# jdfxzzy/DPMN

Measured on AMD Instinct MI355X. Metric: SR images/sec (16x64->32x128, bs=48 per GPU, fp32 forward), higher is better.
Workload: dtype f32; 1 GPU; cfg1: TATT PSN + 3+3 PGRM (embed 96, windows 2/4/8) + CMM, forward-only; per_gpu_batch=48, global_batch=48, ranks=1, batches_in_flight=2, parallelism=dp1 (independent batch shards, no forward collective)

## Files before the change

### dpmn_amd/_abi.py

```python
import ctypes as C
import os

import torch

_HERE = os.path.dirname(os.path.abspath(__file__))
LIB_PATH = os.environ.get("DPMN_HIP_LIB") or os.path.join(_HERE, "lib", "libdpmn_hip.so")

if not os.path.exists(LIB_PATH):
    raise RuntimeError(
        "dpmn_amd: %s not found -- build it with `python -c 'import __graft_entry__ as g; g.build()'` "
        "(or `make -C dpmn_amd/csrc`).  There is no CPU fallback for the DPMN hot path." % LIB_PATH)

lib = C.CDLL(LIB_PATH)

fp = C.c_void_p


class PgrmBlock(C.Structure):
    _fields_ = [(n, fp) for n in (
        "norm1_q_w", "norm1_q_b", "norm1_kv_w", "norm1_kv_b", "q_w", "q_b", "kv_w", "kv_b")] + [
        ("bias_table", fp * 4)] + [(n, fp) for n in (
            "sk_proj_w", "sk_proj_b", "sk_fc1_w", "sk_fc1_b", "sk_fc2_w", "sk_fc2_b", "sk_head_w", "sk_head_b",
            "norm2_w", "norm2_b", "fc1_w", "fc1_b", "dw_w", "dw_b", "pw_w", "pw_b", "fc2_w", "fc2_b")]

# ... 118 lines not shown
    "dpmn_distill_forward_f32": (_i, [C.POINTER(DistillParams), fp, fp, _i, fp, fp, fp, fp, fp, _sz, _i, _i, _i, fp]),
    "dpmn_distill_backward_f32": (_i, [C.POINTER(DistillParams), C.POINTER(DistillGrads), fp, fp, fp, fp, fp, fp, fp, fp, fp, _sz, _i, _i, _i, fp]),
    "dpmn_conv2d_wgrad_unpack_multi_f32": (_i, [fp, fp, _i, _i, fp]),
    "dpmn_tl_interp_f32": (_i, [fp, fp, _i, _i, _i, _i, _i, fp]),
    "dpmn_pointwise_wgrad_det_bytes": (_sz, [_i, _i]),
    "dpmn_reduce_defer_begin": (_i, []),
    "dpmn_reduce_defer_enable": (_i, [_i]),
    "dpmn_reduce_defer_push": (_i, [C.POINTER(TnPending)]),
    "dpmn_reduce_defer_pending": (_i, []),
    "dpmn_reduce_defer_flush": (_i, [_i, fp]),
    "dpmn_xred_fallbacks": (_i, [C.POINTER(C.c_uint), _i]),
    "dpmn_selftest_xshfl": (_i, [C.POINTER(C.c_uint)]),
    "dpmn_selftest_lds_poison": (_i, [C.c_uint, _i, fp]),
    "dpmn_xred_test_force_recompute": (_i, [_i]),
    "dpmn_xred_enable": (_i, [_i]),
    "dpmn_nchw_to_nhwc_f32": (_i, [fp, fp, _i, _i, _i, _i, _i, fp]),
    "dpmn_nhwc_to_nchw_f32": (_i, [fp, fp, _i, _i, _i, _i, fp]),
    "dpmn_se_gate_f32": (_i, [fp, fp, fp, fp, fp, fp, fp, _i, _i, _i, _i, fp]),
    "dpmn_bigru_f32": (_i, [fp, fp, fp, fp, fp, _i, _i, _i, C.c_long, C.c_long, C.c_long, _i, fp]),
    "dpmn_small_linear_f32": (_i, [fp, fp, _i, fp, fp, fp, _i, _i, _i, _i, _f, fp]),
    "dpmn_tatt_encoder_layer_f32": (_i, [fp, fp, _PP, fp, _i, _i, _i, _i, fp]),
    "dpmn_cross_attn_f32": (_i, [fp, fp, fp, fp, fp, _i, _i, _i, _i, _i, fp]),
    "dpmn_add_layernorm64_f32": (_i, [fp, fp, fp, fp, fp, fp, fp, fp, _f, _i, C.c_long, fp]),
    "dpmn_gru_gate_f32": (_i, [fp, fp, fp, fp, C.c_long, _i, _i, fp]),
    "dpmn_to_mask_f32": (_i, [fp, C.c_long, fp, _i, _i, _i, fp]),
    "dpmn_mha32_f32": (_i, [fp, fp, _i, _i, _i, _f, fp]),
    "dpmn_layernorm_std_f32": (_i, [fp, fp, fp, _f, fp, _l, _i, fp]),
    "dpmn_rotate_img_f32": (_i, [fp, fp, fp, _f, fp, _i, _i, _i, _i, fp]),
    "dpmn_blend_f32": (_i, [fp, C.c_long, fp, C.c_long, fp, _f, _i, _i, fp]),
    "dpmn_psnr_ssim_workspace_bytes": (_sz, [_i, _i, _i, _i]),
    "dpmn_psnr_ssim_f32": (_i, [fp, C.c_long, fp, C.c_long, fp, fp, _i, _i, _i, _i, fp]),
    "dpmn_gemm_tn_f32": (_i, [fp, fp, fp, fp, _i, _i, _i, fp, _sz, fp]),
    "dpmn_gemm_tn_partial_bytes": (_sz, [_i, _i, _i]),
    "dpmn_gemm_tn_partial_f32": (_i, [fp, fp, fp, fp, _i, _i, _i, fp, _sz, C.POINTER(TnPending), fp]),
    "dpmn_tn_reduce_multi_f32": (_i, [C.POINTER(TnPending), _i, fp]),
    "dpmn_gemm_tn_group_f32": (_i, [C.POINTER(TnItem), _i, fp]),
    "dpmn_colsum_f32": (_i, [fp, fp, C.c_long, _i, fp]),
    "dpmn_colsum_det_f32": (_i, [fp, fp, C.c_long, _i, fp, _sz, fp]),
    "dpmn_layernorm_bwd_f32": (_i, [fp, fp, fp, _f, fp, _i, fp, fp, C.c_long, _i, fp]),
    "dpmn_layernorm_bwd_det_f32": (_i, [fp, fp, fp, _f, fp, _i, fp, fp, C.c_long, _i, fp, _sz, fp]),
    "dpmn_layernorm_bwd_det_drop_f32": (_i, [fp, fp, fp, _f, fp, _i, fp, fp, C.c_long, _i, fp, _sz, fp, _f, _u64, _f, _u64, _l, fp]),
    "dpmn_layernorm_f32": (_i, [fp, fp, fp, _f, fp, C.c_long, _i, fp]),
    "dpmn_act_bwd_f32": (_i, [fp, fp, fp, _i, _f, C.c_long, fp]),
    "dpmn_act_fwd_f32": (_i, [fp, fp, _i, _f, C.c_long, fp]),
    "dpmn_axpby_f32": (_i, [fp, fp, fp, _f, _f, _i, C.c_long, fp]),
    "dpmn_rowsum_mod_f32": (_i, [fp, fp, C.c_long, _i, _i, fp]),
# ... 234 lines not shown
```

### dpmn_amd/csrc/common.h

```cpp
#pragma once
#include <hip/hip_runtime.h>
#include <stdint.h>
#include <atomic>
#include "../../include/dpmn_hip.h"

typedef float f32x4 __attribute__((ext_vector_type(4)));

#define DPMN_CHECK_LAUNCH()                                                         \
  do {                                                                              \
    hipError_t e__ = hipGetLastError();                                             \
    if (e__ != hipSuccess) return dpmn_set_error(DPMN_ERR_LAUNCH, hipGetErrorString(e__)); \
  } while (0)

#define DPMN_REQUIRE(cond, msg)                                    \
  do {                                                             \
    if (!(cond)) return dpmn_set_error(DPMN_ERR_ARG, msg);         \
  } while (0)

int dpmn_set_error(int code, const char* msg);

__device__ __forceinline__ f32x4 mfma16(float a, float b, f32x4 c) {
  return __builtin_amdgcn_mfma_f32_16x16x4f32(a, b, c, 0, 0, 0);
}

// ... 121 lines not shown
  return u >= p ? inv_keep : 0.0f;
}
__device__ __forceinline__ float drop_scale(unsigned long long seed, unsigned long long idx, float p, float inv_keep) {
  return drop_scale_z(drop_z0(seed, idx), p, inv_keep);
}

static inline hipStream_t as_stream(dpmn_stream_t s) { return (hipStream_t)s; }

constexpr int DPMN_MAX_DEVICES = 64;
int dpmn_cu_count();
template <auto Kernel>
inline void dpmn_lds_optin(size_t bytes) {
  static std::atomic<int> set[DPMN_MAX_DEVICES];
  int dev = -1;
  const bool keyed = hipGetDevice(&dev) == hipSuccess && dev >= 0 && dev < DPMN_MAX_DEVICES;
  if (keyed && (int)bytes <= set[dev].load(std::memory_order_relaxed)) return;
  if (hipFuncSetAttribute(reinterpret_cast<const void*>(Kernel), hipFuncAttributeMaxDynamicSharedMemorySize, (int)bytes) == hipSuccess && keyed)
    set[dev].store((int)bytes, std::memory_order_relaxed);
}

enum ProfTag { PT_CONV_IGEMM_128 = 0, PT_CONV_IGEMM_64, PT_CONV_IGEMM_NARROW, PT_CONV_SPLITK_REDUCE, PT_CONV_HALO, PT_CONV_HALO_C4,
               PT_GEMM_PW, PT_GEMM_WSTAT, PT_GEMM_KLOOP, PT_DWCONV_GELU, PT_WATTN8, PT_WATTN_SCALAR, PT_ATTN_FUSED, PT_BIGRU,
               PT_MHA32, PT_PATCH_EMBED, PT_SK_GATE, PT_TAIL, PT_GEMM_WSTAT_LN, PT_CONV_IGEMM_SK, PT_ATTN_FUSED_BWD, PT_WATTN_BWD,
               PT_CONV_WGRAD, PT_GEMM_TN, PT_TN_REDUCE, PT_DWCONV_BWD, PT_WGRAD_UNPACK, PT_CONV_PACK, PT_AFFINE_ACT_BWD, PT_LN_BWD, PT_WATTN_MFMA32, PT_COUNT };
extern unsigned long long g_dpmn_prof_mask;
extern double g_dpmn_prof_hint_bytes;
extern int g_dpmn_bf16;
extern int g_dpmn_x3;
typedef __bf16 bf16x2 __attribute__((ext_vector_type(2)));
typedef __bf16 bf16x8 __attribute__((ext_vector_type(8)));
__device__ __forceinline__ uint2 pack_bf16x4(float a, float b, float c, float d) {
  typedef float f32x2_ __attribute__((ext_vector_type(2)));
  const bf16x2 lo = __builtin_convertvector((f32x2_){a, b}, bf16x2), hi = __builtin_convertvector((f32x2_){c, d}, bf16x2);
  return make_uint2(__builtin_bit_cast(unsigned, lo), __builtin_bit_cast(unsigned, hi));
}
__device__ __forceinline__ f32x4 mfma16_bf16(bf16x8 a, bf16x8 b, f32x4 c) {
  return __builtin_amdgcn_mfma_f32_16x16x32_bf16(a, b, c, 0, 0, 0);
}
__device__ __forceinline__ void x3_split2t(float a, float b, unsigned& h, unsigned& m, unsigned& l) {
  const unsigned ua = __float_as_uint(a), ub = __float_as_uint(b);
  h = __builtin_amdgcn_perm(ub, ua, 0x07060302u);
  const float ra = a - __uint_as_float(ua & 0xffff0000u), rb = b - __uint_as_float(ub & 0xffff0000u);
  const unsigned va = __float_as_uint(ra), vb = __float_as_uint(rb);
  m = __builtin_amdgcn_perm(vb, va, 0x07060302u);
  const float sa = ra - __uint_as_float(va & 0xffff0000u), sb = rb - __uint_as_float(vb & 0xffff0000u);
  l = __builtin_amdgcn_perm(__float_as_uint(sb), __float_as_uint(sa), 0x07060302u);
}
// ... 24 lines not shown
```

### dpmn_amd/csrc/psn_forward.hip

```cpp
#include "common.h"

namespace {
struct PsnWs {
  float *r1, *r2, *gi, *s, *f[2], *t, *u;
  size_t total;
};
PsnWs carve(const dpmn_psn_weights* w, int B, int H, int W, char* base) {
  size_t off = 0;
  auto take = [&](size_t n) {
    float* p = base ? reinterpret_cast<float*>(base + off) : nullptr;
    off += ((n * sizeof(float) + 255) / 256) * 256;
    return p;
  };
  const size_t px = (size_t)B * H * W, ch = w->ch;
  PsnWs s;
  s.r1 = take(px * ch); s.r2 = take(px * ch); s.gi = take(px * 6 * w->hidden); s.s = take(px * ch);
  s.f[0] = take(px * ch); s.f[1] = take(px * ch); s.t = take(px * ch); s.u = take(px * 4 * ch);
  s.total = off;
  return s;
}
dpmn_conv_desc conv_same(const float* in, int cin, int B, int H, int W, int k, const float* wp, const float* bias, int cout, float* out,
                         const dpmn_cmm_scratch* sc) {
  dpmn_conv_desc d{};
  d.in[0] = in; d.cseg[0] = cin;
// ... 76 lines not shown
}

extern "C" {

size_t dpmn_tatt_interpreter_workspace_bytes(int B, int L, int S) {
  if (B <= 0 || L <= 0 || S <= 0) return 0;
  return carve_tpi(B, L, S, 64, nullptr).total;
}

int dpmn_tatt_interpreter_f32(const dpmn_tatt_interp_weights* w, const float* x, int t_emb, const float* b1, const float* qe,
                              const float* pos, float* tp, float* pw, void* workspace, size_t workspace_bytes, int B, int L, int S,
                              dpmn_stream_t stream) {
  DPMN_REQUIRE(w && x && b1 && qe && pos && tp && workspace, "tatt_interpreter: null pointer");
  DPMN_REQUIRE(w->n_dec >= 1 && w->n_dec <= 4 && w->nhead > 0, "tatt_interpreter: 1..4 decoder layers");
  const int E = 64;
  TpiWs s = carve_tpi(B, L, S, E, static_cast<char*>(workspace));
  if (s.total > workspace_bytes) return dpmn_set_error(DPMN_ERR_WORKSPACE, "tatt_interpreter: workspace too small");
  const int BL = B * L, BS = B * S;
  int rc;
#define RUN(call) do { rc = (call); if (rc != DPMN_OK) return rc; } while (0)
  RUN(dpmn_small_linear_f32(x, nullptr, 0, w->fc_in_w, w->fc_in_b, s.src, BS, E, t_emb, DPMN_ACT_PRELU, w->fc_in_slope, stream));
  RUN(dpmn_tatt_encoder_layer_f32(s.src, pos, w->enc, s.mem, B, S, E, w->nhead, stream));
  const float* out = b1;
  for (int li = 0; li < w->n_dec; ++li) {
    const dpmn_tatt_dec_layer& d = w->dec[li];
    const bool last = li == w->n_dec - 1;
    RUN(dpmn_add_linear_f32(out, qe, d.wq, d.bq, s.q, BL, E, E, DPMN_ACT_NONE, stream));
    RUN(dpmn_small_linear_f32(s.mem, pos, S, d.wk, d.bk, s.k, BS, E, E, DPMN_ACT_NONE, 0.f, stream));
    RUN(dpmn_small_linear_f32(s.mem, nullptr, 0, d.wv, d.bv, s.v, BS, E, E, DPMN_ACT_NONE, 0.f, stream));
    RUN(dpmn_cross_attn_f32(s.q, s.k, s.v, s.o, last ? pw : nullptr, B, L, S, E, w->nhead, stream));
    RUN(dpmn_linear_f32(s.o, d.out_w, d.out_b, out, nullptr, s.t1, BL, E, E, DPMN_ACT_NONE, 0.f, stream));
    float* o1 = s.out[0];
    RUN(dpmn_add_layernorm64_f32(s.t1, nullptr, d.norm2_w, d.norm2_b, o1, nullptr, nullptr, nullptr, 1.0f, 0, BL, stream));
    RUN(dpmn_linear_f32(o1, d.lin1_w, d.lin1_b, nullptr, nullptr, s.f, BL, E, E, DPMN_ACT_RELU, 0.f, stream));
    RUN(dpmn_linear_f32(s.f, d.lin2_w, d.lin2_b, o1, nullptr, s.t1, BL, E, E, DPMN_ACT_NONE, 0.f, stream));
    float* o2 = s.out[1];
    RUN(dpmn_add_layernorm64_f32(s.t1, nullptr, d.norm3_w, d.norm3_b, o2, w->dec_norm_w, w->dec_norm_b, tp, 1.0f / w->n_dec, li > 0 ? 1 : 0,
                                 BL, stream));
    out = o2;
  }
#undef RUN
  return DPMN_OK;
}

}
```

### dpmn_amd/csrc/runtime.hip

```cpp
#include "common.h"
#include <string.h>
#include <stdlib.h>

static thread_local char g_err[512] = "";

int dpmn_set_error(int code, const char* msg) {
  strncpy(g_err, msg ? msg : "", sizeof(g_err) - 1);
  g_err[sizeof(g_err) - 1] = 0;
  return code;
}

int dpmn_cu_count() {
  static std::atomic<int> cus[DPMN_MAX_DEVICES];
  int dev = -1;
  if (hipGetDevice(&dev) != hipSuccess) return 256;
  const bool keyed = dev >= 0 && dev < DPMN_MAX_DEVICES;
  int n = keyed ? cus[dev].load(std::memory_order_relaxed) : 0;
  if (n < 1) {
    if (hipDeviceGetAttribute(&n, hipDeviceAttributeMultiprocessorCount, dev) != hipSuccess || n < 1) return 256;
    if (keyed) cus[dev].store(n, std::memory_order_relaxed);
  }
  return n;
}

unsigned long long g_dpmn_prof_mask = 0ull;
double g_dpmn_prof_hint_bytes = 0.0;
int g_dpmn_x3 = 0;
int g_dpmn_bf16 = 0;
namespace {
const char* const kTagNames[PT_COUNT] = {
    "k_conv_igemm<128,128>", "k_conv_igemm<64,64>", "k_conv_igemm<128,16|32>", "k_conv_splitk_reduce", "k_conv_halo", "k_conv_halo_c4",
    "k_gemm_pw", "k_gemm_wstat|rowreg", "k_gemm_kloop", "k_dwconv_gelu", "k_window_attn8_mfma", "k_window_attn<2|4>", "k_ln_qkv_window_attn",
    "k_bigru", "k_mha32", "k_patch_embed_ln", "k_sk_gate", "k_tail_conv2", "k_gemm_wstat|rowreg<LN prologue>", "k_conv_igemm_sk", "k_ln_qkv_window_attn_bwd", "k_window_attn_bwd_mfma",
    "k_conv_wgrad", "k_gemm_tn_reg", "k_tn_reduce_multi", "k_dwconv_bwd", "k_wgrad_unpack_multi", "k_conv_pack_multi", "k_affine_act_bwd", "k_ln_bwd", "k_window_attn_mfma<4|8|16,32>"};
struct Rec { int tag; double flops, bytes; };
struct Prof {
  int cap = 0, count = 0, limit = 0;
  hipEvent_t* ev = nullptr;
  Rec* rec = nullptr;
} g_prof;
}

int dpmn_prof_open(int tag, hipStream_t st, double flops, double bytes) {
  if (g_prof.count >= g_prof.limit) return -1;
  const int i = g_prof.count++;
  g_prof.rec[i] = Rec{tag, flops, bytes};
  (void)hipEventRecord(g_prof.ev[2 * i], st);
  return i;
}
void dpmn_prof_close(int slot, hipStream_t st) { (void)hipEventRecord(g_prof.ev[2 * slot + 1], st); }

extern "C" {
int dpmn_abi_version(void) { return 5; }
int dpmn_set_compute_dtype(int mode) {
  DPMN_REQUIRE(mode >= 0 && mode <= 2, "set_compute_dtype: 0 = f32, 1 = bf16 operands, 2 = f32 via three bf16 terms");
  g_dpmn_bf16 = mode == 1;
  g_dpmn_x3 = mode == 2;
// ... 46 lines not shown
```

### dpmn_amd/csrc/tatt.hip

```cpp
#include "common.h"

namespace {

typedef float v2f __attribute__((ext_vector_type(2)));

template <int HID>
__global__ __launch_bounds__(256) void k_bigru(const float* gi, const float* w_hh ,
                                                const float* b_hh , const float* res,
                                                float* out, int nseq, int T, int inner, long outer_stride,
                                                long inner_stride, long step_stride) {
  static_assert(HID == 32, "lane mapping assumes 32 hidden units per direction");
  __shared__ __attribute__((aligned(16))) float hs[4][64];
  const int wave = threadIdx.x >> 6, lane = threadIdx.x & 63;
  const int dir = lane >> 5, j = lane & 31;
  const long s = (long)blockIdx.x * 4 + wave;
  if (s >= nseq) return;
  v2f wrz[HID], wnn[HID / 2];
  const float* wb = w_hh + (size_t)dir * 3 * HID * HID;
#pragma unroll
  for (int k = 0; k < HID; ++k) wrz[k] = v2f{wb[(size_t)j * HID + k], wb[(size_t)(HID + j) * HID + k]};
#pragma unroll
  for (int k = 0; k < HID / 2; ++k) wnn[k] = v2f{wb[(size_t)(2 * HID + j) * HID + 2 * k], wb[(size_t)(2 * HID + j) * HID + 2 * k + 1]};
  const float br = b_hh[dir * 3 * HID + j], bz = b_hh[dir * 3 * HID + HID + j], bn = b_hh[dir * 3 * HID + 2 * HID + j];
  asm volatile("" ::: "memory");
// ... 283 lines not shown
__global__ __launch_bounds__(256) void k_add_layernorm64(const float* __restrict__ x, const float* __restrict__ res,
                                                          const float* __restrict__ g, const float* __restrict__ b,
                                                          float* __restrict__ y, const float* __restrict__ g2,
                                                          const float* __restrict__ b2, float* __restrict__ acc_out, float alpha,
                                                          int accumulate, long M) {
  const long row = (long)blockIdx.x * 4 + (threadIdx.x >> 6);
  const int lane = threadIdx.x & 63;
  if (row >= M) return;
  float v = x[row * 64 + lane] + (res ? res[row * 64 + lane] : 0.f);
  float mean = wave_sum(v) * (1.0f / 64);
  float d = v - mean;
  float var = wave_sum(d * d) * (1.0f / 64);
  const float o = d * (1.0f / sqrtf(var + 1e-5f)) * g[lane] + b[lane];
  y[row * 64 + lane] = o;
  if (acc_out) {
    mean = wave_sum(o) * (1.0f / 64);
    d = o - mean;
    var = wave_sum(d * d) * (1.0f / 64);
    const float o2 = (d * (1.0f / sqrtf(var + 1e-5f)) * g2[lane] + b2[lane]) * alpha;
    acc_out[row * 64 + lane] = accumulate ? acc_out[row * 64 + lane] + o2 : o2;
  }
}

__global__ void k_gru_gate(const float* __restrict__ gi, const float* __restrict__ gh, float* __restrict__ h,
                           float* __restrict__ hist, long hist_row_stride, int R, int H) {
  const long idx = (long)blockIdx.x * blockDim.x + threadIdx.x;
  if (idx >= (long)R * H) return;
  const int r_ = idx / H, j = idx % H;
  const float* a = gi + (size_t)r_ * 3 * H;
  const float* c = gh + (size_t)r_ * 3 * H;
  const float r = sigmoid_f(a[j] + c[j]);
  const float z = sigmoid_f(a[H + j] + c[H + j]);
  const float n = tanhf(a[2 * H + j] + r * c[2 * H + j]);
  const float hn = (1.f - z) * n + z * h[idx];
  h[idx] = hn;
  hist[(size_t)r_ * hist_row_stride + j] = hn;
}

__global__ void k_tl_interp(const float* __restrict__ in, float* __restrict__ out, int N, int Win, int C, int H, int W) {
  const long idx = (long)blockIdx.x * blockDim.x + threadIdx.x;
  const int c4 = C / 4;
  if (idx >= (long)N * H * W * c4) return;
  const int c = (idx % c4) * 4;
  const int x = (idx / c4) % W, n = idx / ((long)c4 * W * H);
  const float sx = W > 1 ? (float)x * ((float)(Win - 1) / (float)(W - 1)) : 0.f;
  int x0 = (int)sx;
// ... 23 lines not shown
int dpmn_small_linear_f32(const float* x, const float* add, int add_rows, const float* w, const float* b, float* y, int M,
                          int N, int K, int act, float slope, dpmn_stream_t stream) {
  DPMN_REQUIRE(x && w && y && M > 0 && N > 0 && K > 0, "small_linear: bad arguments");
  hipLaunchKernelGGL(k_small_linear_tiled, dim3((unsigned)((M + 31) / 32), (unsigned)((N + 63) / 64)), dim3(256), 0, as_stream(stream), x,
                     add, add_rows > 0 ? add_rows : 1, w, b, y, M, N, K, act, slope);
  DPMN_CHECK_LAUNCH();
  return DPMN_OK;
}

int dpmn_tatt_encoder_layer_f32(const float* src, const float* pos, const float* const* w12, float* mem, int N, int L,
                                int E, int nhead, dpmn_stream_t stream) {
  DPMN_REQUIRE(src && pos && w12 && mem && N > 0, "encoder_layer: bad arguments");
  DPMN_REQUIRE(E == 64 && nhead == 4 && L <= 32, "encoder_layer: built for d_model=64, 4 heads, <=32 tokens (tatt.py:171-178)");
  EncW w{w12[0], w12[1], w12[2], w12[3], w12[4], w12[5], w12[6], w12[7], w12[8], w12[9], w12[10], w12[11]};
  hipLaunchKernelGGL((k_encoder_layer<64, 4>), dim3(N), dim3(256), 0, as_stream(stream), src, pos, w, mem, L);
  DPMN_CHECK_LAUNCH();
  return DPMN_OK;
}

int dpmn_cross_attn_f32(const float* q, const float* k, const float* v, float* o, float* pw, int N, int L, int S, int E,
                        int nhead, dpmn_stream_t stream) {
  DPMN_REQUIRE(q && k && v && o && N > 0, "cross_attn: bad arguments");
  DPMN_REQUIRE(E == 64 && nhead == 4 && S <= 32, "cross_attn: built for d_model=64, 4 heads, <=32 keys");
  hipLaunchKernelGGL((k_cross_attn<64, 4>), dim3(cdiv(L, 256), N), dim3(256), 0, as_stream(stream), q, k, v, o, pw, L, S);
  DPMN_CHECK_LAUNCH();
  return DPMN_OK;
}

int dpmn_add_layernorm64_f32(const float* x, const float* res, const float* g, const float* b, float* y, const float* g2,
                             const float* b2, float* acc_out, float alpha, int accumulate, long M, dpmn_stream_t stream) {
  DPMN_REQUIRE(x && g && b && y && M > 0, "add_layernorm64: bad arguments");
  DPMN_REQUIRE(!acc_out || (g2 && b2), "add_layernorm64: second norm parameters required with acc_out");
  hipLaunchKernelGGL(k_add_layernorm64, dim3((unsigned)((M + 3) / 4)), dim3(256), 0, as_stream(stream), x, res, g, b, y, g2, b2,
                     acc_out, alpha, accumulate, M);
  DPMN_CHECK_LAUNCH();
  return DPMN_OK;
}

int dpmn_gru_gate_f32(const float* gi, const float* gh, float* h, float* hist, long hist_row_stride, int R, int H,
                      dpmn_stream_t stream) {
  DPMN_REQUIRE(gi && gh && h && hist && R > 0 && H > 0, "gru_gate: bad arguments");
  const long total = (long)R * H;
  hipLaunchKernelGGL(k_gru_gate, dim3((unsigned)((total + 255) / 256)), dim3(256), 0, as_stream(stream), gi, gh, h, hist,
                     hist_row_stride, R, H);
  DPMN_CHECK_LAUNCH();
  return DPMN_OK;
}
// ... 11 lines not shown
```

### dpmn_amd/model/tatt.py

```python
import math

import torch
from .._abi import stream_of as _abi_stream_of
import torch.nn as nn

from .. import ops
from .tsrn import _PSNBase


class _EncLayer(nn.Module):
    def __init__(self, d, nhead, ff):
        super().__init__()
        self.self_attn = nn.MultiheadAttention(d, nhead)
        self.linear1 = nn.Linear(d, ff)
        self.linear2 = nn.Linear(ff, d)
        self.norm1 = nn.LayerNorm(d)
        self.norm2 = nn.LayerNorm(d)


class _DecLayer(nn.Module):
    def __init__(self, d, nhead, ff):
        super().__init__()
        self.self_attn = nn.MultiheadAttention(d, nhead)
        self.multihead_attn = nn.MultiheadAttention(d, nhead)
# ... 133 lines not shown
            w = self._interp_native(P)
            pos = ig.pe.pe[0, :S].contiguous()
            qe = self._query_embed(B, b1.device)
            tp = torch.empty(B * L, E, device=b1.device)
            pw = torch.empty(B, L, S, device=b1.device) if self.need_pr_weights else None
            if not hasattr(self, "_interp_ws"):
                self._interp_ws = {}
            key = (B, L, S, _abi_stream_of(b1.device))
            if key not in self._interp_ws:
                self._interp_ws[key] = torch.empty(lib.dpmn_tatt_interpreter_workspace_bytes(B, L, S) // 4, device=b1.device)
            ws = self._interp_ws[key]
            check(lib.dpmn_tatt_interpreter_f32(_C.byref(w), dptr(x), x.shape[2], dptr(b1), dptr(qe), dptr(pos), dptr(tp), dptr(pw, True),
                                                dptr(ws), ws.numel() * 4, B, L, S, stream()))
            return tp.reshape(B, H, W, E), pw
        src = ops.small_linear(x.reshape(B * S, -1), ig.fc_in.weight, ig.fc_in.bias, act="prelu", slope=P["fc_in_slope"])
        pos = ig.pe.pe[0, :S].contiguous()
        mem = ops.tatt_encoder_layer(src.reshape(B, S, E), pos, P["enc"]).reshape(B * S, E)
        qe = self._query_embed(B, b1.device).reshape(B * L, E)
        out = b1.reshape(B * L, E)
        tp = torch.empty(B * L, E, device=b1.device)
        dn = ig.upsample_transformer.decoder.norm
        pw = None
        layers = ig.upsample_transformer.decoder.layers
        for li, (d, pk) in enumerate(zip(layers, P["dec"])):
            q = ops.add_linear(out, qe, pk["wq"], pk["bq"])
            k = ops.small_linear(mem, pk["wk"], pk["bk"], add=pos)
            v = ops.small_linear(mem, pk["wv"], pk["bv"])
            last = li == len(layers) - 1
            o, w_ = ops.cross_attn(q.reshape(B, L, E), k.reshape(B, S, E), v.reshape(B, S, E),
                                   need_weights=last and self.need_pr_weights)
            pw = w_ if last else pw
            t1 = ops.linear(o.reshape(B * L, E), d.multihead_attn.out_proj.weight, d.multihead_attn.out_proj.bias, res1=out)
            out = ops.add_layernorm64(t1, None, d.norm2.weight, d.norm2.bias)
            f = ops.linear(out, d.linear1.weight, d.linear1.bias, act="relu")
            t2 = ops.linear(f, d.linear2.weight, d.linear2.bias, res1=out)
            out = ops.add_layernorm64(t2, None, d.norm3.weight, d.norm3.bias, dn.weight, dn.bias, tp,
                                      alpha=1.0 / len(layers), accumulate=li > 0)
        return tp.reshape(B, H, W, E), pw

    def forward(self, x, text_emb=None, text_emb_gt=None, feature_arcs=None, rand_offs=None):
        self._check_mode()
        P = self._trunk_pack()
        if text_emb is None:
            text_emb = torch.zeros(1, 37, 1, 26, device=x.device)
        if text_emb.shape[0] != x.shape[0]:
            raise ValueError("TATT: text_emb batch must match the image batch")
        b1 = self._head(x, P)
        tp_map, prw = self._tp_interpreter(b1, text_emb, P)
        return self._trunk(b1, P, tp_map), prw
```

### dpmn_amd/ops.py

```python
import torch
from ._abi import stream_of as _abi_stream_of

from . import _abi
from ._abi import dptr, lib, check, stream

ACT = {"none": 0, "gelu": 1, "relu": 2, "leaky02": 3, "leaky001": 4, "mish": 5, "prelu": 6, "tanh": 7, "sigmoid": 8,
       "relu_post_res": 9}


def linear(x, w, bias=None, res1=None, res2=None, act="none", slope=0.0):
    M, K = x.shape
    N = w.shape[0]
    y = torch.empty(M, N, device=x.device)
    check(lib.dpmn_linear_f32(dptr(x), dptr(w), dptr(bias, True), dptr(res1, True), dptr(res2, True), dptr(y), M, N, K,
                              ACT[act], float(slope), stream()))
    return y


def add_linear(x, addv, w, bias=None, act="none"):
    M, K = x.shape
    N = w.shape[0]
    y = torch.empty(M, N, device=x.device)
    check(lib.dpmn_add_linear_f32(dptr(x), dptr(addv), dptr(w), dptr(bias, True), dptr(y), M, N, K, ACT[act], stream()))
    return y
# ... 1134 lines not shown
    N, L, E = src.shape
    mem = torch.empty_like(src)
    check(lib.dpmn_tatt_encoder_layer_f32(dptr(src), dptr(pos), _abi.ptr_array(w12), dptr(mem), N, L, E, nhead, stream()))
    return mem


def cross_attn(q, k, v, nhead=4, need_weights=False):
    N, L, E = q.shape
    S = k.shape[1]
    o = torch.empty_like(q)
    pw = torch.empty(N, L, S, device=q.device) if need_weights else None
    check(lib.dpmn_cross_attn_f32(dptr(q), dptr(k), dptr(v), dptr(o), dptr(pw, True), N, L, S, E, nhead, stream()))
    return o, pw


def add_layernorm64(x, res, g, b, g2=None, b2=None, acc_out=None, alpha=1.0, accumulate=False):
    M = x.numel() // 64
    y = torch.empty_like(x)
    check(lib.dpmn_add_layernorm64_f32(dptr(x), dptr(res, True), dptr(g), dptr(b), dptr(y), dptr(g2, True), dptr(b2, True),
                                       dptr(acc_out, True), float(alpha), int(accumulate), M, stream()))
    return y


def gru_gate(gi, gh, h, hist, hist_row_stride):
    R, H = h.shape
    check(lib.dpmn_gru_gate_f32(dptr(gi), dptr(gh), dptr(h), hist.data_ptr(), hist_row_stride, R, H, stream()))


def _nchw_view(x):
    if not x.is_cuda or x.dtype != torch.float32:
        raise _abi.DpmnError("dpmn_amd: expected a float32 CUDA tensor")
    B, Cc, H, W = x.shape
    if x.stride()[1:] != (H * W, W, 1):
        x = x.contiguous()
    return x, x.data_ptr(), x.stride(0)


def to_mask(img):
    img, p, st = _nchw_view(img)
    B, _, H, W = img.shape
    out = torch.empty(B, 3, H, W, device=img.device)
    check(lib.dpmn_to_mask_f32(p, st, dptr(out), B, H, W, stream()))
    return out


def mha32(qkv, B, L, heads, scale):
# ... 346 lines not shown
```

### include/dpmn_hip.h

```cpp
#ifndef DPMN_HIP_H
#define DPMN_HIP_H

#include <stddef.h>
#include <stdint.h>

#ifdef __cplusplus
extern "C" {
#endif

typedef void* dpmn_stream_t;

enum { DPMN_OK = 0, DPMN_ERR_ARG = -1, DPMN_ERR_LAUNCH = -2, DPMN_ERR_WORKSPACE = -3, DPMN_ERR_RUNTIME = -4 };

enum { DPMN_ACT_NONE = 0, DPMN_ACT_GELU = 1, DPMN_ACT_RELU = 2, DPMN_ACT_LEAKY02 = 3, DPMN_ACT_LEAKY001 = 4,
       DPMN_ACT_MISH = 5, DPMN_ACT_PRELU = 6, DPMN_ACT_TANH = 7, DPMN_ACT_SIGMOID = 8,
       DPMN_ACT_RELU_POST_RES = 9  };

int dpmn_abi_version(void);
const char* dpmn_last_error(void);
int dpmn_set_compute_dtype(int mode);
int dpmn_get_compute_dtype(void);

int dpmn_linear_f32(const float* x, const float* w, const float* bias, const float* res1, const float* res2,
                    float* y, int M, int N, int K, int act, float slope, dpmn_stream_t stream);
// ... 526 lines not shown
  const float *g2_w, *g2_b, *g2_whh, *g2_bhh;
} dpmn_psn_srb;
typedef struct {
  int in_planes, ch, hidden, srb_nums;
  dpmn_psn_srb srb[8];
  const float *b7_w, *b7_b, *up_w, *up_b, *last_w, *last_b;
} dpmn_psn_weights;
size_t dpmn_psn_trunk_workspace_bytes(const dpmn_psn_weights* w, int B, int H, int W);
int dpmn_psn_trunk_f32(const dpmn_psn_weights* w, const float* b1, const float* tp, int tp_channels, float* out, void* workspace,
                       size_t workspace_bytes, const dpmn_cmm_scratch* scratch, int B, int H, int W, dpmn_stream_t stream);

typedef struct {
  const float *wq, *bq, *wk, *bk, *wv, *bv;
  const float *out_w, *out_b, *norm2_w, *norm2_b, *lin1_w, *lin1_b, *lin2_w, *lin2_b, *norm3_w, *norm3_b;
} dpmn_tatt_dec_layer;
typedef struct {
  int n_dec, nhead;
  const float *fc_in_w, *fc_in_b;
  float fc_in_slope;
  const float* enc[12];
  dpmn_tatt_dec_layer dec[4];
  const float *dec_norm_w, *dec_norm_b;
} dpmn_tatt_interp_weights;
size_t dpmn_tatt_interpreter_workspace_bytes(int B, int L, int S);
int dpmn_tatt_interpreter_f32(const dpmn_tatt_interp_weights* w, const float* x, int t_emb, const float* b1, const float* qe,
                              const float* pos, float* tp, float* pw, void* workspace, size_t workspace_bytes, int B, int L, int S,
                              dpmn_stream_t stream);

#ifdef __cplusplus
}
#endif
#endif
```

Measured before the change: 6427 images/s.

## Fuse TATT decoder Q-projection into cross-attention and fuse decoder tail MLP/LayerNorms

Folds the query projection (x+qe times Wq) into the cross-attention kernel using MFMA, and replaces the per-layer decoder tail (out_proj, add+LN, linear1+ReLU, linear2, add+LN, final decoder norm and tp accumulation) with one persistent kernel that keeps weights in LDS and rows in registers. The aim is to cut kernel launches and the global-memory round trips of intermediate activations in the TATT decoder. In exchange it adds specialised code paths limited to E=64, 4 heads and S<=32, plus more LDS per block, which may lower occupancy.

```diff
diff --git a/dpmn_amd/_abi.py b/dpmn_amd/_abi.py
--- a/dpmn_amd/_abi.py
+++ b/dpmn_amd/_abi.py
@@ -164,6 +164,8 @@
     "dpmn_tatt_encoder_layer_f32": (_i, [fp, fp, _PP, fp, _i, _i, _i, _i, fp]),
     "dpmn_cross_attn_f32": (_i, [fp, fp, fp, fp, fp, _i, _i, _i, _i, _i, fp]),
     "dpmn_add_layernorm64_f32": (_i, [fp, fp, fp, fp, fp, fp, fp, fp, _f, _i, C.c_long, fp]),
+    "dpmn_cross_attn_qproj_f32": (_i, [fp, fp, fp, fp, fp, fp, fp, fp, _i, _i, _i, _i, _i, fp]),
+    "dpmn_tatt_dec_tail_f32": (_i, [fp, fp, C.POINTER(TattDecLayer), fp, fp, fp, fp, _f, _i, C.c_long, fp]),
     "dpmn_gru_gate_f32": (_i, [fp, fp, fp, fp, C.c_long, _i, _i, fp]),
     "dpmn_to_mask_f32": (_i, [fp, C.c_long, fp, _i, _i, _i, fp]),
     "dpmn_mha32_f32": (_i, [fp, fp, _i, _i, _i, _f, fp]),
diff --git a/dpmn_amd/csrc/common.h b/dpmn_amd/csrc/common.h
--- a/dpmn_amd/csrc/common.h
+++ b/dpmn_amd/csrc/common.h
@@ -167,7 +167,8 @@
 enum ProfTag { PT_CONV_IGEMM_128 = 0, PT_CONV_IGEMM_64, PT_CONV_IGEMM_NARROW, PT_CONV_SPLITK_REDUCE, PT_CONV_HALO, PT_CONV_HALO_C4,
                PT_GEMM_PW, PT_GEMM_WSTAT, PT_GEMM_KLOOP, PT_DWCONV_GELU, PT_WATTN8, PT_WATTN_SCALAR, PT_ATTN_FUSED, PT_BIGRU,
                PT_MHA32, PT_PATCH_EMBED, PT_SK_GATE, PT_TAIL, PT_GEMM_WSTAT_LN, PT_CONV_IGEMM_SK, PT_ATTN_FUSED_BWD, PT_WATTN_BWD,
-               PT_CONV_WGRAD, PT_GEMM_TN, PT_TN_REDUCE, PT_DWCONV_BWD, PT_WGRAD_UNPACK, PT_CONV_PACK, PT_AFFINE_ACT_BWD, PT_LN_BWD, PT_WATTN_MFMA32, PT_COUNT };
+               PT_CONV_WGRAD, PT_GEMM_TN, PT_TN_REDUCE, PT_DWCONV_BWD, PT_WGRAD_UNPACK, PT_CONV_PACK, PT_AFFINE_ACT_BWD, PT_LN_BWD, PT_WATTN_MFMA32, PT_CROSS_ATTN,
+               PT_TATT_DEC_TAIL, PT_COUNT };
 extern unsigned long long g_dpmn_prof_mask;
 extern double g_dpmn_prof_hint_bytes;
 extern int g_dpmn_bf16;
diff --git a/dpmn_amd/csrc/psn_forward.hip b/dpmn_amd/csrc/psn_forward.hip
--- a/dpmn_amd/csrc/psn_forward.hip
+++ b/dpmn_amd/csrc/psn_forward.hip
@@ -122,9 +122,19 @@
   RUN(dpmn_small_linear_f32(x, nullptr, 0, w->fc_in_w, w->fc_in_b, s.src, BS, E, t_emb, DPMN_ACT_PRELU, w->fc_in_slope, stream));
   RUN(dpmn_tatt_encoder_layer_f32(s.src, pos, w->enc, s.mem, B, S, E, w->nhead, stream));
   const float* out = b1;
+  const bool fused = E == 64 && w->nhead == 4 && S <= 32;
   for (int li = 0; li < w->n_dec; ++li) {
     const dpmn_tatt_dec_layer& d = w->dec[li];
     const bool last = li == w->n_dec - 1;
+    if (fused) {
+      RUN(dpmn_small_linear_f32(s.mem, pos, S, d.wk, d.bk, s.k, BS, E, E, DPMN_ACT_NONE, 0.f, stream));
+      RUN(dpmn_small_linear_f32(s.mem, nullptr, 0, d.wv, d.bv, s.v, BS, E, E, DPMN_ACT_NONE, 0.f, stream));
+      RUN(dpmn_cross_attn_qproj_f32(out, qe, d.wq, d.bq, s.k, s.v, s.o, last ? pw : nullptr, B, L, S, E, w->nhead, stream));
+      float* o2 = s.out[li & 1];
+      RUN(dpmn_tatt_dec_tail_f32(s.o, out, &d, o2, w->dec_norm_w, w->dec_norm_b, tp, 1.0f / w->n_dec, li > 0 ? 1 : 0, BL, stream));
+      out = o2;
+      continue;
+    }
     RUN(dpmn_add_linear_f32(out, qe, d.wq, d.bq, s.q, BL, E, E, DPMN_ACT_NONE, stream));
     RUN(dpmn_small_linear_f32(s.mem, pos, S, d.wk, d.bk, s.k, BS, E, E, DPMN_ACT_NONE, 0.f, stream));
     RUN(dpmn_small_linear_f32(s.mem, nullptr, 0, d.wv, d.bv, s.v, BS, E, E, DPMN_ACT_NONE, 0.f, stream));
diff --git a/dpmn_amd/csrc/runtime.hip b/dpmn_amd/csrc/runtime.hip
--- a/dpmn_amd/csrc/runtime.hip
+++ b/dpmn_amd/csrc/runtime.hip
@@ -32,7 +32,8 @@
     "k_conv_igemm<128,128>", "k_conv_igemm<64,64>", "k_conv_igemm<128,16|32>", "k_conv_splitk_reduce", "k_conv_halo", "k_conv_halo_c4",
     "k_gemm_pw", "k_gemm_wstat|rowreg", "k_gemm_kloop", "k_dwconv_gelu", "k_window_attn8_mfma", "k_window_attn<2|4>", "k_ln_qkv_window_attn",
     "k_bigru", "k_mha32", "k_patch_embed_ln", "k_sk_gate", "k_tail_conv2", "k_gemm_wstat|rowreg<LN prologue>", "k_conv_igemm_sk", "k_ln_qkv_window_attn_bwd", "k_window_attn_bwd_mfma",
-    "k_conv_wgrad", "k_gemm_tn_reg", "k_tn_reduce_multi", "k_dwconv_bwd", "k_wgrad_unpack_multi", "k_conv_pack_multi", "k_affine_act_bwd", "k_ln_bwd", "k_window_attn_mfma<4|8|16,32>"};
+    "k_conv_wgrad", "k_gemm_tn_reg", "k_tn_reduce_multi", "k_dwconv_bwd", "k_wgrad_unpack_multi", "k_conv_pack_multi", "k_affine_act_bwd", "k_ln_bwd", "k_window_attn_mfma<4|8|16,32>", "k_cross_attn",
+    "k_tatt_dec_tail"};
 struct Rec { int tag; double flops, bytes; };
 struct Prof {
   int cap = 0, count = 0, limit = 0;
diff --git a/dpmn_amd/csrc/tatt.hip b/dpmn_amd/csrc/tatt.hip
--- a/dpmn_amd/csrc/tatt.hip
+++ b/dpmn_amd/csrc/tatt.hip
@@ -329,6 +329,261 @@
   }
 }
 
+struct DecTailW {
+  const float *out_w, *out_b, *n2_w, *n2_b, *l1_w, *l1_b, *l2_w, *l2_b, *n3_w, *n3_b, *dn_w, *dn_b;
+};
+constexpr int DT_LDW = 64 + 4;
+constexpr size_t DT_SMEM = (size_t)(3 * 64 * DT_LDW + 9 * 64) * sizeof(float);
+template <int E, int ACC>
+__global__ __launch_bounds__(256, 2) void k_tatt_dec_tail(const float* __restrict__ o, const float* res, DecTailW w, float* y,
+                                                          float* acc_out, float alpha, int M) {
+  static_assert(E == 64, "built for d_model = 64: four 16-wide k chunks = four 16-wide n tiles");
+  constexpr int KC = E / 16, NT = E / 16, LDW = DT_LDW;
+  extern __shared__ __attribute__((aligned(16))) float smem[];
+  float* Ws = smem;
+  float* pv = Ws + 3 * E * LDW;
+  const int tid = threadIdx.x, wave = tid >> 6, lane = tid & 63, lr = lane & 15, kq = lane >> 4;
+  const int tiles = (M + 15) / 16;
+  const int stride = gridDim.x * 4;
+  int tile = blockIdx.x * 4 + wave;
+  auto row_of = [&](int t_) -> size_t {
+    const int m = (t_ < tiles ? t_ : tiles - 1) * 16 + lr;
+    return (size_t)(m < M ? m : M - 1);
+  };
+  f32x4 xr[KC], rr[NT], ta[NT];
+  auto load_rows = [&](int t_) {
+    const float* p = o + row_of(t_) * E + 4 * kq;
+#pragma unroll
+    for (int c = 0; c < KC; ++c) xr[c] = *reinterpret_cast<const f32x4*>(p + 16 * c);
+  };
+  auto load_res = [&](int t_) {
+    const size_t ro = row_of(t_) * E + 4 * kq;
+#pragma unroll
+    for (int nt = 0; nt < NT; ++nt) {
+      rr[nt] = *reinterpret_cast<const f32x4*>(res + ro + 16 * nt);
+      if (ACC == 2) ta[nt] = *reinterpret_cast<const f32x4*>(acc_out + ro + 16 * nt);
+    }
+  };
+  load_rows(tile);
+  load_res(tile);
+  for (int i = tid; i < 3 * E * (E / 4); i += 256) {
+    const int mat = i / (E * (E / 4)), j = i % (E * (E / 4)), r = j / (E / 4), c4 = (j % (E / 4)) * 4;
+    const float* src = mat == 0 ? w.out_w : (mat == 1 ? w.l1_w : w.l2_w);
+    *reinterpret_cast<float4*>(Ws + (mat * E + r) * LDW + c4) = *reinterpret_cast<const float4*>(src + (size_t)r * E + c4);
+  }
+  if (tid < E) {
+    pv[tid] = w.out_b[tid]; pv[E + tid] = w.l1_b[tid]; pv[2 * E + tid] = w.l2_b[tid];
+    pv[3 * E + tid] = w.n2_w[tid]; pv[4 * E + tid] = w.n2_b[tid]; pv[5 * E + tid] = w.n3_w[tid]; pv[6 * E + tid] = w.n3_b[tid];
+    if (ACC) { pv[7 * E + tid] = w.dn_w[tid]; pv[8 * E + tid] = w.dn_b[tid]; }
+  }
+  __syncthreads();
+
+  auto mm = [&](const float* W, const f32x4 (&b)[KC], f32x4 (&acc)[NT]) {
+#pragma unroll
+    for (int nt = 0; nt < NT; ++nt) acc[nt] = (f32x4){0.f, 0.f, 0.f, 0.f};
+    const float* wa = W + lr * LDW + 4 * kq;
+    f32x4 wf[2][NT];
+#pragma unroll
+    for (int nt = 0; nt < NT; ++nt) wf[0][nt] = *reinterpret_cast<const f32x4*>(wa + 16 * nt * LDW);
+#pragma unroll
+    for (int c = 0; c < KC; ++c) {
+      if (c + 1 < KC) {
+#pragma unroll
+        for (int nt = 0; nt < NT; ++nt) wf[(c + 1) & 1][nt] = *reinterpret_cast<const f32x4*>(wa + 16 * nt * LDW + 16 * (c + 1));
+      }
+#pragma unroll
+      for (int s4 = 0; s4 < 4; ++s4)
+#pragma unroll
+        for (int nt = 0; nt < NT; ++nt) acc[nt] = mfma16(wf[c & 1][nt][s4], b[c][s4], acc[nt]);
+      __builtin_amdgcn_sched_barrier(0);
+    }
+  };
+  auto ln = [&](f32x4 (&v)[NT], const float* g, const float* b) {
+    float s0 = 0.f, s1 = 0.f;
+#pragma unroll
+    for (int nt = 0; nt < NT; ++nt) { s0 += v[nt][0] + v[nt][1]; s1 += v[nt][2] + v[nt][3]; }
+    float s_ = s0 + s1;
+    s_ += xshfl<16>(s_); s_ += xshfl<32>(s_);
+    const float mean = s_ * (1.0f / E);
+    float q0 = 0.f, q1 = 0.f, q2 = 0.f, q3 = 0.f;
+#pragma unroll
+    for (int nt = 0; nt < NT; ++nt) {
+      v[nt][0] -= mean; v[nt][1] -= mean; v[nt][2] -= mean; v[nt][3] -= mean;
+      q0 = fmaf(v[nt][0], v[nt][0], q0); q1 = fmaf(v[nt][1], v[nt][1], q1); q2 = fmaf(v[nt][2], v[nt][2], q2); q3 = fmaf(v[nt][3], v[nt][3], q3);
+    }
+    float q = (q0 + q1) + (q2 + q3);
+    q += xshfl<16>(q); q += xshfl<32>(q);
+    const float rstd = 1.0f / sqrtf(q * (1.0f / E) + 1e-5f);
+#pragma unroll
+    for (int nt = 0; nt < NT; ++nt) {
+      const f32x4 g4 = *reinterpret_cast<const f32x4*>(g + 16 * nt + 4 * kq), b4 = *reinterpret_cast<const f32x4*>(b + 16 * nt + 4 * kq);
+#pragma unroll
+      for (int r = 0; r < 4; ++r) v[nt][r] = v[nt][r] * rstd * g4[r] + b4[r];
+    }
+  };
+
+  for (; tile < tiles; tile += stride) {
+    const size_t off = row_of(tile) * E + 4 * kq;
+    f32x4 xb[KC], acc[NT], h[NT], tc[NT];
+#pragma unroll
+    for (int c = 0; c < KC; ++c) xb[c] = xr[c];
+    __builtin_amdgcn_sched_barrier(0);
+    load_rows(tile + stride);
+    __builtin_amdgcn_sched_barrier(0);
+    mm(Ws, xb, acc);
+#pragma unroll
+    for (int nt = 0; nt < NT; ++nt) {
+      h[nt] = acc[nt] + *reinterpret_cast<const f32x4*>(pv + 16 * nt + 4 * kq) + rr[nt];
+      if (ACC == 2) tc[nt] = ta[nt];
+    }
+    __builtin_amdgcn_sched_barrier(0);
+    load_res(tile + stride);
+    __builtin_amdgcn_sched_barrier(0);
+    ln(h, pv + 3 * E, pv + 4 * E);
+    mm(Ws + E * LDW, h, acc);
+#pragma unroll
+    for (int nt = 0; nt < NT; ++nt) {
+      const f32x4 b4 = *reinterpret_cast<const f32x4*>(pv + E + 16 * nt + 4 * kq);
+#pragma unroll
+      for (int r = 0; r < 4; ++r) { const float a = acc[nt][r] + b4[r]; xb[nt][r] = a > 0.f ? a : 0.f; }
+    }
+    mm(Ws + 2 * E * LDW, xb, acc);
+#pragma unroll
+    for (int nt = 0; nt < NT; ++nt) h[nt] = acc[nt] + *reinterpret_cast<const f32x4*>(pv + 2 * E + 16 * nt + 4 * kq) + h[nt];
+    ln(h, pv + 5 * E, pv + 6 * E);
+#pragma unroll
+    for (int nt = 0; nt < NT; ++nt) *reinterpret_cast<f32x4*>(y + off + 16 * nt) = h[nt];
+    if (ACC) {
+      ln(h, pv + 7 * E, pv + 8 * E);
+#pragma unroll
+      for (int nt = 0; nt < NT; ++nt) {
+        f32x4 v = h[nt] * alpha;
+        if (ACC == 2) v = tc[nt] + v;
+        *reinterpret_cast<f32x4*>(acc_out + off + 16 * nt) = v;
+      }
+    }
+  }
+}
+
+constexpr int CA_LDQ = 64 + 4;
+constexpr size_t CA_SMEM = (size_t)(2 * 32 * 64 + 64 * CA_LDQ + 64 + 4 * 64 * CA_LDQ) * sizeof(float);
+template <int E, int NH>
+__global__ __launch_bounds__(256) void k_cross_attn_qproj(const float* __restrict__ x, const float* __restrict__ qe,
+                                                           const float* __restrict__ wq, const float* __restrict__ bq,
+                                                           const float* __restrict__ k, const float* __restrict__ v,
+                                                           float* __restrict__ o, float* __restrict__ pw, int L, int S) {
+  static_assert(E == 64, "built for d_model = 64");
+  constexpr int SMAX = 32, D = E / NH, KC = E / 16, NT = E / 16, LDQ = CA_LDQ;
+  extern __shared__ __attribute__((aligned(16))) float smem[];
+  float (*Ks)[E] = reinterpret_cast<float (*)[E]>(smem);
+  float (*Vs)[E] = reinterpret_cast<float (*)[E]>(smem + SMAX * E);
+  float* Wq = smem + 2 * SMAX * E;
+  float* bqs = Wq + E * LDQ;
+  const int n = blockIdx.y, tid = threadIdx.x, wave = tid >> 6, lane = tid & 63, lr = lane & 15, kq = lane >> 4;
+  float* Q = bqs + E + wave * 64 * LDQ;
+  const int l0 = blockIdx.x * 256 + wave * 64;
+  f32x4 xa[4][KC], qa[4][KC];
+#pragma unroll
+  for (int mt = 0; mt < 4; ++mt) {
+    const int lq = l0 + 16 * mt + lr;
+    const size_t ro = ((size_t)n * L + (lq < L ? lq : L - 1)) * E + 4 * kq;
+#pragma unroll
+    for (int c = 0; c < KC; ++c) {
+      xa[mt][c] = *reinterpret_cast<const f32x4*>(x + ro + 16 * c);
+      qa[mt][c] = *reinterpret_cast<const f32x4*>(qe + ro + 16 * c);
+    }
+  }
+  for (int i = tid; i < S * E; i += 256) {
+    Ks[i / E][i % E] = k[(size_t)n * S * E + i];
+    Vs[i / E][i % E] = v[(size_t)n * S * E + i];
+  }
+  for (int i = tid; i < E * (E / 4); i += 256) {
+    const int r = i / (E / 4), c4 = (i % (E / 4)) * 4;
+    *reinterpret_cast<float4*>(Wq + r * LDQ + c4) = *reinterpret_cast<const float4*>(wq + (size_t)r * E + c4);
+  }
+  if (tid < E) bqs[tid] = bq ? bq[tid] : 0.f;
+  __syncthreads();
+  if (l0 >= L) return;
+  {
+    const float* wa = Wq + lr * LDQ + 4 * kq;
+#pragma unroll
+    for (int mt = 0; mt < 4; ++mt) {
+      f32x4 acc[NT];
+#pragma unroll
+      for (int nt = 0; nt < NT; ++nt) acc[nt] = (f32x4){0.f, 0.f, 0.f, 0.f};
+#pragma unroll
+      for (int c = 0; c < KC; ++c) {
+        const f32x4 xb = xa[mt][c] + qa[mt][c];
+        f32x4 wf[NT];
+#pragma unroll
+        for (int nt = 0; nt < NT; ++nt) wf[nt] = *reinterpret_cast<const f32x4*>(wa + 16 * nt * LDQ + 16 * c);
+#pragma unroll
+        for (int s4 = 0; s4 < 4; ++s4)
+#pragma unroll
+          for (int nt = 0; nt < NT; ++nt) acc[nt] = mfma16(wf[nt][s4], xb[s4], acc[nt]);
+      }
+#pragma unroll
+      for (int nt = 0; nt < NT; ++nt)
+        *reinterpret_cast<f32x4*>(Q + (16 * mt + lr) * LDQ + 16 * nt + 4 * kq) = acc[nt] + *reinterpret_cast<const f32x4*>(bqs + 16 * nt + 4 * kq);
+    }
+  }
+  __builtin_amdgcn_wave_barrier();
+  const int l = l0 + lane;
+  if (l >= L) return;
+  const float* qr = Q + lane * LDQ;
+  float* orow = o + ((size_t)n * L + l) * E;
+  const float scale = 1.0f / sqrtf((float)D);
+  float pavg[SMAX];
+#pragma unroll
+  for (int s = 0; s < SMAX; ++s) pavg[s] = 0.f;
+#pragma unroll
+  for (int hh = 0; hh < NH; ++hh) {
+    float qv[D];
+#pragma unroll
+    for (int d = 0; d < D; d += 4) {
+      const float4 t4 = *reinterpret_cast<const float4*>(qr + hh * D + d);
+      qv[d] = t4.x * scale; qv[d + 1] = t4.y * scale; qv[d + 2] = t4.z * scale; qv[d + 3] = t4.w * scale;
+    }
+    float sc[SMAX];
+    float mx = -INFINITY;
+#pragma unroll
+    for (int s = 0; s < SMAX; ++s) {
+      float a = -INFINITY;
+      if (s < S) {
+        a = 0.f;
+#pragma unroll
+        for (int d = 0; d < D; ++d) a += qv[d] * Ks[s][hh * D + d];
+      }
+      sc[s] = a;
+      mx = fmaxf(mx, a);
+    }
+    float den = 0.f;
+#pragma unroll
+    for (int s = 0; s < SMAX; ++s) { sc[s] = (s < S) ? expf(sc[s] - mx) : 0.f; den += sc[s]; }
+    const float inv = 1.0f / den;
+    float acc[D];
+#pragma unroll
+    for (int d = 0; d < D; ++d) acc[d] = 0.f;
+#pragma unroll
+    for (int s = 0; s < SMAX; ++s) {
+      const float p = sc[s] * inv;
+      pavg[s] += p;
+      if (s < S) {
+#pragma unroll
+        for (int d = 0; d < D; ++d) acc[d] += p * Vs[s][hh * D + d];
+      }
+    }
+#pragma unroll
+    for (int d = 0; d < D; d += 4)
+      *reinterpret_cast<float4*>(orow + hh * D + d) = make_float4(acc[d], acc[d + 1], acc[d + 2], acc[d + 3]);
+  }
+  if (pw) {
+    float* pr = pw + ((size_t)n * L + l) * S;
+#pragma unroll
+    for (int s = 0; s < SMAX; ++s) if (s < S) pr[s] = pavg[s] * (1.0f / NH);
+  }
+}
+
 __global__ void k_gru_gate(const float* __restrict__ gi, const float* __restrict__ gh, float* __restrict__ h,
                            float* __restrict__ hist, long hist_row_stride, int R, int H) {
   const long idx = (long)blockIdx.x * blockDim.x + threadIdx.x;
@@ -398,7 +653,49 @@
                         int nhead, dpmn_stream_t stream) {
   DPMN_REQUIRE(q && k && v && o && N > 0, "cross_attn: bad arguments");
   DPMN_REQUIRE(E == 64 && nhead == 4 && S <= 32, "cross_attn: built for d_model=64, 4 heads, <=32 keys");
+  ProfScope prof(PT_CROSS_ATTN, as_stream(stream), 4.0 * N * (double)L * S * E,
+                 4.0 * (2.0 * N * (double)L * E + 2.0 * N * (double)S * E + (pw ? (double)N * L * S : 0.0)));
   hipLaunchKernelGGL((k_cross_attn<64, 4>), dim3(cdiv(L, 256), N), dim3(256), 0, as_stream(stream), q, k, v, o, pw, L, S);
+  DPMN_CHECK_LAUNCH();
+  return DPMN_OK;
+}
+
+int dpmn_cross_attn_qproj_f32(const float* x, const float* qe, const float* wq, const float* bq, const float* k, const float* v,
+                              float* o, float* pw, int N, int L, int S, int E, int nhead, dpmn_stream_t stream) {
+  DPMN_REQUIRE(x && qe && wq && k && v && o && N > 0 && L > 0 && S > 0, "cross_attn_qproj: bad arguments");
+  DPMN_REQUIRE(E == 64 && nhead == 4 && S <= 32, "cross_attn_qproj: built for d_model=64, 4 heads, <=32 keys");
+  ProfScope prof(PT_CROSS_ATTN, as_stream(stream), 4.0 * N * (double)L * S * E + 2.0 * N * (double)L * E * E,
+                 4.0 * (3.0 * N * (double)L * E + 2.0 * N * (double)S * E + (double)E * E + (pw ? (double)N * L * S : 0.0)));
+  dpmn_lds_optin<k_cross_attn_qproj<64, 4>>(CA_SMEM);
+  hipLaunchKernelGGL((k_cross_attn_qproj<64, 4>), dim3(cdiv(L, 256), N), dim3(256), CA_SMEM, as_stream(stream), x, qe, wq, bq, k, v, o,
+                     pw, L, S);
+  DPMN_CHECK_LAUNCH();
+  return DPMN_OK;
+}
+
+int dpmn_tatt_dec_tail_f32(const float* o, const float* res, const dpmn_tatt_dec_layer* d, float* y, const float* g2, const float* b2,
+                           float* acc_out, float alpha, int accumulate, long M, dpmn_stream_t stream) {
+  DPMN_REQUIRE(o && res && d && y && M > 0 && M <= (1L << 30), "tatt_dec_tail: bad arguments");
+  DPMN_REQUIRE(d->out_w && d->out_b && d->norm2_w && d->norm2_b && d->lin1_w && d->lin1_b && d->lin2_w && d->lin2_b && d->norm3_w && d->norm3_b,
+               "tatt_dec_tail: null layer parameter");
+  DPMN_REQUIRE(!acc_out || (g2 && b2), "tatt_dec_tail: second norm parameters required with acc_out");
+  const DecTailW w{d->out_w, d->out_b, d->norm2_w, d->norm2_b, d->lin1_w, d->lin1_b, d->lin2_w, d->lin2_b, d->norm3_w, d->norm3_b, g2, b2};
+  const int tiles = (int)((M + 15) / 16), cus = dpmn_cu_count();
+  int gx = 2 * cus;
+  while (gx > cus && (long)gx * 4 * 3 > tiles) gx -= cus;
+  if (gx * 4 > tiles) gx = cdiv(tiles, 4);
+  const int mode = !acc_out ? 0 : (accumulate ? 2 : 1);
+  ProfScope prof(PT_TATT_DEC_TAIL, as_stream(stream), 3.0 * 2.0 * (double)M * 64 * 64, 4.0 * (double)M * 64 * (mode == 0 ? 3 : (mode == 1 ? 4 : 5)));
+#define DPMN_DT_LAUNCH(ACC)                                                                                                        \
+  do {                                                                                                                             \
+    dpmn_lds_optin<k_tatt_dec_tail<64, ACC>>(DT_SMEM);                                                                             \
+    hipLaunchKernelGGL((k_tatt_dec_tail<64, ACC>), dim3(gx), dim3(256), DT_SMEM, as_stream(stream), o, res, w, y, acc_out, alpha, \
+                       (int)M);                                                                                                    \
+  } while (0)
+  if (mode == 0) DPMN_DT_LAUNCH(0);
+  else if (mode == 1) DPMN_DT_LAUNCH(1);
+  else DPMN_DT_LAUNCH(2);
+#undef DPMN_DT_LAUNCH
   DPMN_CHECK_LAUNCH();
   return DPMN_OK;
 }
diff --git a/dpmn_amd/model/tatt.py b/dpmn_amd/model/tatt.py
--- a/dpmn_amd/model/tatt.py
+++ b/dpmn_amd/model/tatt.py
@@ -179,11 +179,20 @@
         dn = ig.upsample_transformer.decoder.norm
         pw = None
         layers = ig.upsample_transformer.decoder.layers
+        fused = E == 64 and S <= 32
         for li, (d, pk) in enumerate(zip(layers, P["dec"])):
-            q = ops.add_linear(out, qe, pk["wq"], pk["bq"])
             k = ops.small_linear(mem, pk["wk"], pk["bk"], add=pos)
             v = ops.small_linear(mem, pk["wv"], pk["bv"])
             last = li == len(layers) - 1
+            if fused:
+                o, w_ = ops.cross_attn_qproj(out.reshape(B, L, E), qe.reshape(B, L, E), pk["wq"], pk["bq"], k.reshape(B, S, E),
+                                             v.reshape(B, S, E), need_weights=last and self.need_pr_weights)
+                pw = w_ if last else pw
+                out = ops.tatt_dec_tail(o.reshape(B * L, E), out, d.multihead_attn.out_proj.weight, d.multihead_attn.out_proj.bias,
+                                        d.norm2.weight, d.norm2.bias, d.linear1.weight, d.linear1.bias, d.linear2.weight, d.linear2.bias,
+                                        d.norm3.weight, d.norm3.bias, dn.weight, dn.bias, tp, alpha=1.0 / len(layers), accumulate=li > 0)
+                continue
+            q = ops.add_linear(out, qe, pk["wq"], pk["bq"])
             o, w_ = ops.cross_attn(q.reshape(B, L, E), k.reshape(B, S, E), v.reshape(B, S, E),
                                    need_weights=last and self.need_pr_weights)
             pw = w_ if last else pw
diff --git a/dpmn_amd/ops.py b/dpmn_amd/ops.py
--- a/dpmn_amd/ops.py
+++ b/dpmn_amd/ops.py
@@ -1180,6 +1180,29 @@
     return y
 
 
+def cross_attn_qproj(x, qe, wq, bq, k, v, nhead=4, need_weights=False):
+    N, L, E = x.shape
+    S = k.shape[1]
+    o = torch.empty_like(x)
+    pw = torch.empty(N, L, S, device=x.device) if need_weights else None
+    check(lib.dpmn_cross_attn_qproj_f32(dptr(x), dptr(qe), dptr(wq), dptr(bq, True), dptr(k), dptr(v), dptr(o), dptr(pw, True),
+                                        N, L, S, E, nhead, stream()))
+    return o, pw
+
+
+def tatt_dec_tail(o, res, out_w, out_b, n2_w, n2_b, l1_w, l1_b, l2_w, l2_b, n3_w, n3_b, g2=None, b2=None, acc_out=None, alpha=1.0,
+                  accumulate=False):
+    M = o.numel() // 64
+    d = _abi.TattDecLayer()
+    for n, t in (("out_w", out_w), ("out_b", out_b), ("norm2_w", n2_w), ("norm2_b", n2_b), ("lin1_w", l1_w), ("lin1_b", l1_b),
+                 ("lin2_w", l2_w), ("lin2_b", l2_b), ("norm3_w", n3_w), ("norm3_b", n3_b)):
+        setattr(d, n, dptr(t))
+    y = torch.empty_like(o)
+    check(lib.dpmn_tatt_dec_tail_f32(dptr(o), dptr(res), _abi.C.byref(d), dptr(y), dptr(g2, True), dptr(b2, True), dptr(acc_out, True),
+                                     float(alpha), int(accumulate), M, stream()))
+    return y
+
+
 def gru_gate(gi, gh, h, hist, hist_row_stride):
     R, H = h.shape
     check(lib.dpmn_gru_gate_f32(dptr(gi), dptr(gh), dptr(h), hist.data_ptr(), hist_row_stride, R, H, stream()))
diff --git a/include/dpmn_hip.h b/include/dpmn_hip.h
--- a/include/dpmn_hip.h
+++ b/include/dpmn_hip.h
@@ -572,6 +572,10 @@
   dpmn_tatt_dec_layer dec[4];
   const float *dec_norm_w, *dec_norm_b;
 } dpmn_tatt_interp_weights;
+int dpmn_tatt_dec_tail_f32(const float* o, const float* res, const dpmn_tatt_dec_layer* d, float* y, const float* g2, const float* b2,
+                           float* acc_out, float alpha, int accumulate, long M, dpmn_stream_t stream);
+int dpmn_cross_attn_qproj_f32(const float* x, const float* qe, const float* wq, const float* bq, const float* k, const float* v,
+                              float* o, float* pw, int N, int L, int S, int E, int nhead, dpmn_stream_t stream);
 size_t dpmn_tatt_interpreter_workspace_bytes(int B, int L, int S);
 int dpmn_tatt_interpreter_f32(const dpmn_tatt_interp_weights* w, const float* x, int t_emb, const float* b1, const float* qe,
                               const float* pos, float* tp, float* pw, void* workspace, size_t workspace_bytes, int B, int L, int S,
```

Result: faster. 6562 images/s (median of 6 runs) (+2.1%).
